# wgurecky/CORRLA_RS

Hardware: AMD Instinct MI355X
Metric: RSVD GFLOP/s on 16k x 16k f32 rank-128 (higher is better)
Workload: dtype f32

## Files before the change

corrla_rs_amd/csrc/driver.hpp:

```cpp
#pragma once
#include <cstdio>
#include <chrono>
#include <cmath>
#include <cstdint>
#include <cstring>
#include <limits>
#include <stdexcept>
#include <string>
#include <functional>
#include <vector>

#include "gemm_plan.hpp"
#include "small_linalg.hpp"

namespace corrla {

struct Error : std::runtime_error {
  int code;
  Error(int c, const std::string& m) : std::runtime_error(m), code(c) {}
};
enum { ST_OK = 0, ST_EINVAL = 1, ST_ENOMEM = 2, ST_EHIP = 3, ST_ECOMM = 4, ST_ENUMERIC = 5, ST_ENODEV = 6 };

inline int64_t round_up(int64_t x, int64_t a) { return (x + a - 1) / a * a; }

// ... 85 lines not shown
  bool qr_householder = false;
  static constexpr const T* kNone = nullptr;

  explicit RsvdDriver(Dev& d, bool profile = false) : dev(d), profile_phases(profile) {}

  int mixed_planes_ = 0;
  void a_times(const TallA<T>& a, const Skinny<T>& x, Skinny<T>& y, const T* scale_dev) {
    if (mixed_planes_ && dev.template mixed_fits<T>(!a.row_major, a.mem, x, y))
      dev.gemm_mixed(!a.row_major, a.mem, x, y, scale_dev, mixed_planes_), ++tm.n_mixed_products;
    else if (a.row_major)
      dev.gemm_nn(a.mem, x, y, scale_dev);
    else
      dev.gemm_tn(a.mem, x, y, scale_dev);
    if (a.mu_short || a.mu_tall) {
      T* v = dev.template alloc_scalar<T>((int)x.cols_alloc);
      dev.weighted_colsum(x, a.nt, a.mu_short, v);
      dev.rank1_sub(y, a.mt, a.mu_tall, v, scale_dev);
    }
  }
  void at_times(const TallA<T>& a, const Skinny<T>& y, Skinny<T>& z, const T* scale_dev, bool sharded) {
    if (mixed_planes_ && dev.template mixed_fits<T>(a.row_major, a.mem, y, z))
      dev.gemm_mixed(a.row_major, a.mem, y, z, scale_dev, mixed_planes_), ++tm.n_mixed_products;
    else if (a.row_major)
      dev.gemm_tn(a.mem, y, z, scale_dev);
    else
      dev.gemm_nn(a.mem, y, z, scale_dev);
    if (a.mu_short || a.mu_tall) {
      T* v = dev.template alloc_scalar<T>((int)y.cols_alloc);
      dev.weighted_colsum(y, a.mt, a.mu_tall, v);
      dev.rank1_sub(z, a.nt, a.mu_short, v, scale_dev);
    }
    if (sharded) dev.allreduce(z.p, (size_t)z.ld * (size_t)z.cols);
  }

  static constexpr size_t kStatusBytes = 32;
  int st_slots_ = 0;
  struct Pending {
    int slot, npass;
    bool rough;
    int per_pass;
    void* st = nullptr;
    int st_per_pass = 1;
    bool is_svd = false;
    int flag_slot = -1;
  };
  static constexpr int kRobustPasses = 8;
  bool robust_needs_more_ = false;
  bool svd_needs_more_ = false;
  bool svd_needs_v_ = false;
  bool null_cols_seen_ = false;
  int* flags_pool_ = nullptr;
  int flags_cap_ = 0, flags_used_ = 0;
  bool defer_status_ = false;
  bool optimistic_dirty_ = false;
  void* st_pool_ = nullptr;
  int st_used_ = 0;
  std::vector<Pending> pending_;
  int64_t m_local_ = 0, m_global_ = -1;
  int64_t m_local_override_ = -1;
  int64_t global_rows(bool sharded) {
    if (!sharded) return m_local_;
    if (m_global_ < 0) m_global_ = dev.allreduce_sum_host(m_local_);
    return m_global_;
  }

  int hh_short_shards_ = -1;
// ... 29 lines not shown
    if (const char* e = std::getenv("CORRLA_HH_BLOCK")) wmax = std::max<int64_t>(1, std::min<int64_t>(wmax, std::atoll(e)));
    if (l <= wmax) {
      householder_panel(y, tmp, sharded);
      return;
    }
    const int64_t nb = (l + wmax - 1) / wmax, w = (l + nb - 1) / nb;
    std::vector<double> th;
    for (int64_t c0 = 0; c0 < l; c0 += w) {
      const int64_t wb = std::min(w, l - c0);
      Skinny<T> yb = dev.template alloc_skinny<T>(m, wb), tb = dev.template alloc_skinny<T>(m, wb);
      Skinny<T> pb = dev.template alloc_skinny<T>(m, wb);
      dev.copy_block(y, 0, c0, m, wb, yb, 0, 0);
      for (int pass = 0; pass < 5; ++pass) {
        double overlap2 = 0.0;
        if (c0 > 0) {
          Skinny<T> t = dev.template alloc_skinny<T>(c0, wb);
          dev.gemm_nn(as_rowmajor_transposed(y, c0), yb, t, kNone);
          if (sharded) dev.allreduce(t.p, (size_t)t.ld * (size_t)t.cols_alloc);
          if (pass >= 1) {
            th.resize((size_t)(c0 * wb));
            dev.download_skinny(t, c0, wb, th.data());
            for (double v : th) overlap2 += v * v;
          }
          dev.gemm_tn(as_rowmajor_transposed(y, c0), t, pb, kNone);
          dev.sub_inplace(yb, pb);
        }
        householder_panel(yb, tb, sharded);
        if (c0 == 0 || (pass >= 1 && overlap2 <= 0.25)) break;
      }
      dev.copy_block(yb, 0, 0, m, wb, y, 0, c0);
    }
  }

  int64_t orthonormalize(Skinny<T>& y, Skinny<T>& tmp, bool sharded, bool rough = false) {
    const int64_t l = y.cols;
    if (householder_usable(y, sharded)) {
      PhaseTimer qt0;
      householder_thin_q_any_width(y, tmp, sharded);
      ++tm.qr_passes;
      subphase(tm.qr_gram_ms, qt0);
      return l;
    }
    int64_t r = orthonormalize_core(y, tmp, sharded, rough);
    if (r < l && !defer_status_ && (sharded ? global_rows(true) : y.rows) >= l) r = complete_basis(y, r, sharded);
    return r;
  }

  int64_t complete_basis(Skinny<T>& y, int64_t r, bool sharded) {
    const int64_t l = y.cols, c = l - r, m = y.rows;
    Skinny<T> yc = dev.template alloc_skinny<T>(m, c);
    Skinny<T> pc = dev.template alloc_skinny<T>(m, c);
    Skinny<T> tc = dev.template alloc_skinny<T>(m, c);
    dev.fill_normal(yc.p, m, c, (int64_t)1, yc.ld, (uint64_t)(0x9e3779b97f4a7c15ull ^ (uint64_t)(131 * r + l)), (int64_t)0, c);
    if (r > 0) {
      for (int pass = 0; pass < 2; ++pass) {
        Skinny<T> t = dev.template alloc_skinny<T>(r, c);
        dev.gemm_nn(as_rowmajor_transposed(y, r), yc, t, kNone);
        if (sharded) dev.allreduce(t.p, (size_t)t.ld * (size_t)t.cols_alloc);
        dev.gemm_tn(as_rowmajor_transposed(y, r), t, pc, kNone);
        dev.sub_inplace(yc, pc);
      }
    }
    const int64_t rc = orthonormalize_core(yc, tc, sharded, false);
    dev.copy_cols(yc, y, r, rc);
    return r + rc;
  }

  int64_t orthonormalize_device(Skinny<T>& y, Skinny<T>& tmp, bool sharded, bool rough, bool polish) {
    const int64_t l = y.cols;
    PhaseTimer qt0;
    const bool inplace = dev.qr_inplace_fits(l);
    const bool single = dev.template device_chol_fits<T>(l);
    const int level = std::max(2, std::min(dev.robust_passes(), kRobustPasses));
    const bool inloop = rough && !polish;
    const int npass_even = level;
    const int npass = inloop ? (level <= 2 ? 1 : npass_even - 1) : (polish ? (level <= 2 ? 1 : 3) : level);
    const int always = (polish || inloop) ? 1 : 2;
    int* need = flags_pool_ + flags_used_;
    int* null_mask = dev.alloc_flags((int)l);
    int* need_blk = dev.alloc_flags(2);
    void* st_scratch = dev.alloc_zeroed_bytes((size_t)2 * npass * kStatusBytes);
    void* insp = single ? nullptr : dev.template alloc_inspect<T>();
    Skinny<T> gd = dev.template alloc_skinny<T>(l, l);
    Skinny<T> md = dev.template alloc_skinny<T>(l, l);
    const double eps0 = (double)std::numeric_limits<T>::epsilon();
    double shift_rel = eps0 * std::max({16.0, 0.25 * std::sqrt((double)std::max<int64_t>(y.rows, 1)), single ? 0.0 : 2.0 * (double)l});
    if (const char* e = std::getenv("CORRLA_QR_SHIFT_SCALE")) shift_rel *= std::atof(e);
    float nullx = 1.f;
    if (const char* e = std::getenv("CORRLA_QR_NULL_EXCESS")) nullx = (float)std::atof(e);
    const int64_t n1 = single ? l : round_up((l + 1) / 2, (int64_t)4), n2 = l - n1;
    T* minus_one = nullptr;
    if (!single) {
      minus_one = dev.template alloc_scalar<T>(1);
      dev.fill_const(minus_one, (int64_t)1, (T)-1);
    }
    for (int pass = 0; pass < npass; ++pass) {
      const int gate = pass < always ? -1 : (inplace ? pass - 1 : always + ((pass - always) / 2) * 2 - 1);
      dev.set_run_if(gate < 0 ? nullptr : need + gate);
      Skinny<T> yv = y.view_cols(l);
      dev.gemm_nn(as_rowmajor_transposed(y, l), yv, gd, kNone);
      if (sharded) dev.allreduce(gd.p, (size_t)gd.ld * (size_t)gd.cols_alloc);
      const int shift_mode = polish ? 2 : (pass == 0 ? 1 : 0);
      const float nx = (!polish && pass >= 2) ? nullx : 0.f;
      const float need_ratio = (inloop && pass == 0) ? 1e-2f : 0.f;
      if (single) {
        dev.chol_inv_robust(gd, l, (T)(4.0 * eps0), (float)shift_rel, shift_mode, nx, md, st_scratch, pass, need + pass, null_mask,
                            nullptr, need_ratio);
      } else {
        dev.gram_inspect(gd, l, (float)shift_rel, shift_mode, insp);
        const void* shp = dev.template inspect_shift_ptr<T>(insp);
        Skinny<T> g11 = dev.template alloc_skinny<T>(n1, n1), g12 = dev.template alloc_skinny<T>(n1, n2);
        Skinny<T> g22 = dev.template alloc_skinny<T>(n2, n2), x11 = dev.template alloc_skinny<T>(n1, n1);
        Skinny<T> x22 = dev.template alloc_skinny<T>(n2, n2), r12 = dev.template alloc_skinny<T>(n1, n2);
        Skinny<T> t22 = dev.template alloc_skinny<T>(n2, n2), t12 = dev.template alloc_skinny<T>(n1, n2);
        Skinny<T> x12 = dev.template alloc_skinny<T>(n1, n2);
        dev.copy_block(gd, 0, 0, n1, n1, g11, 0, 0);
        dev.copy_block(gd, 0, n1, n1, n2, g12, 0, 0);
        dev.copy_block(gd, n1, n1, n2, n2, g22, 0, 0);
        dev.chol_inv_robust(g11, n1, (T)(4.0 * eps0), 0.f, 2, nx, x11, st_scratch, 2 * pass, need_blk, null_mask, shp, need_ratio);
        dev.gemm_nn(as_rowmajor_transposed(x11, n1), g12, r12, kNone);
        dev.gemm_nn(as_rowmajor_transposed(r12, n2), r12, t22, kNone);
        dev.sub_inplace(g22, t22);
        dev.chol_inv_robust(g22, n2, (T)(4.0 * eps0), 0.f, 2, nx, x22, st_scratch, 2 * pass + 1, need_blk + 1, null_mask + n1, shp,
                            need_ratio);
        dev.gemm_tn(as_rowmajor_transposed(r12, n2), x22, t12, kNone);
        dev.gemm_tn(as_rowmajor_transposed(x11, n1), t12, x12, minus_one);
        dev.copy_block(x11, 0, 0, n1, n1, md, 0, 0);
        dev.copy_block(x12, 0, 0, n1, n2, md, 0, n1);
        dev.copy_block(x22, 0, 0, n2, n2, md, n1, n1);
        dev.template combine_need<T>(need + pass, need_ratio > 0.f ? nullptr : insp, need_blk, need_blk + 1);
      }
      if (inplace) {
        dev.apply_inplace(y, l, md);
      } else {
        dev.gemm_tn(as_rowmajor_transposed(y, l), md, tmp, kNone);
        std::swap(y.p, tmp.p);
      }
      if (pass + 1 < npass || inloop) dev.refill_null(y, l, null_mask, (uint64_t)(0x9e3779b97f4a7c15ull ^ (uint64_t)(977 * (flags_used_ + pass) + l)));
      if (pass < always) ++tm.qr_passes;
    }
    dev.set_run_if(nullptr);
    Pending pd{always, npass, rough, 0};
    pd.st = st_scratch;
    pd.st_per_pass = single ? 1 : 2;
    pd.flag_slot = (inloop && npass > 1) ? -1 : flags_used_;
    pending_.push_back(pd);
    flags_used_ += npass;
    subphase(tm.qr_gram_ms, qt0);
    return l;
  }

  int64_t orthonormalize_core(Skinny<T>& y, Skinny<T>& tmp, bool sharded, bool rough, bool polish = false) {
    const int64_t l = y.cols;
    int64_t r = l;
    if (defer_status_ && (sharded || y.rows >= l) && flags_used_ + kRobustPasses <= flags_cap_ &&
        dev.template device_qr_robust_fits<T>(l))
      return orthonormalize_device(y, tmp, sharded, rough, polish);
    if (dev.template device_chol_fits<T>(l)) {
      PhaseTimer qt0;
      const int npass = rough ? 1 : 2;
      Skinny<T> gd0 = dev.template alloc_skinny<T>(l, l);
      Skinny<T> md0 = dev.template alloc_skinny<T>(l, l);
      const bool defer = defer_status_ && st_used_ + npass <= st_slots_;
      void* st_dev = defer ? (void*)((char*)st_pool_ + (size_t)st_used_ * kStatusBytes) : dev.alloc_bytes(2 * kStatusBytes);
      const double eps0 = (double)std::numeric_limits<T>::epsilon();
      for (int pass = 0; pass < npass; ++pass) {
        Skinny<T> yv = y.view_cols(l);
        dev.gemm_nn(as_rowmajor_transposed(y, l), yv, gd0, kNone);
        if (sharded) dev.allreduce(gd0.p, (size_t)gd0.ld * (size_t)gd0.cols_alloc);
        dev.chol_inv(gd0, l, (T)(4.0 * eps0), md0, st_dev, pass);
        dev.gemm_tn(as_rowmajor_transposed(y, l), md0, tmp, kNone);
        std::swap(y.p, tmp.p);
        ++tm.qr_passes;
      }
      if (defer) {
        pending_.push_back({st_used_, npass, rough, 1});
        st_used_ += npass;
        subphase(tm.qr_gram_ms, qt0);
        return l;
      }
      int fail[2] = {0, 0};
      float min_ratio[2], dev_i[2];
      dev.read_chol_status(st_dev, npass, fail, min_ratio, dev_i);
      subphase(tm.qr_gram_ms, qt0);
      for (int pass = 0; pass < npass; ++pass)
        if (fail[pass] == 3) throw Error(ST_ENUMERIC, "non-finite Gram matrix in orthonormalisation");
      if (fail[0] == 2) return 0;
      const bool ok = fail[0] == 0 && (rough || (fail[1] == 0 && dev_i[1] <= 0.25f));
      if (ok) return l;
    }
// ... 171 lines not shown
      dev.fill_normal(om.p, a.nt, l, 1, om.ld, o.seed, 0, l);
    }
    Skinny<T> z = dev.template alloc_skinny<T>(a.nt, l);
    double* ss_dev = dev.alloc_f64(1);
    T* inv_dev = dev.template alloc_scalar<T>(1);
    int64_t i0 = 0;
    const bool fused = o.power_fused && n_iter > 0 && a.row_major && !a.mu_short && !a.mu_tall &&
                       dev.template ata_fused_fits<T>(a.mem, l);
    if (fused) {
      const int64_t nf = std::min<int64_t>(n_iter, 3);
      for (int64_t i = 0; i < nf; ++i) {
        if (i == 0) dev.event_mark(0);
        dev.ata_fused(a.mem, i == 0 ? om : z, z);
        if (i == 0) dev.event_mark(1);
        if (o.sharded) dev.allreduce(z.p, (size_t)z.ld * (size_t)z.cols);
        dev.inv_norm(z, ss_dev, inv_dev);
        dev.scale_inplace(z, inv_dev);
        if (i == 0) phase(tm.sketch_ms, pt);
      }
      a_times(a, z, y, kNone);
      i0 = nf;
    } else {
      dev.event_mark(0);
      a_times(a, om, y, kNone);
      dev.event_mark(1);
      phase(tm.sketch_ms, pt);
    }
    for (int64_t i = i0; i < n_iter; ++i) {
      if (i > 2) {
        phase(tm.power_ms, pt);
        orthonormalize(y, y2, o.sharded, true);
        phase(tm.qr_ms, pt);
      }
      at_times(a, y, z, kNone, o.sharded);
      dev.inv_norm(z, ss_dev, inv_dev);
      dev.scale_inplace(z, inv_dev);
      a_times(a, z, y, kNone);
    }
    phase(tm.power_ms, pt);
    int64_t r = orthonormalize(y, y2, o.sharded);
    phase(tm.qr_ms, pt);
    return r;
  }

  void random_svd_tall(const TallA<T>& a, int64_t k, int64_t l, int64_t n_iter, const RunOpts& o, Skinny<T>& u_tall,
                       T* s_dev, Skinny<T>& v_tall, const std::function<void()>& emit = {}) {
    qr_householder = o.qr_householder;
    m_local_ = m_local_override_ >= 0 ? m_local_override_ : a.mt;
    m_global_ = -1;
    hh_short_shards_ = -1;
    const bool hh = qr_householder;
    if (!hh && (dev.template device_chol_fits<T>(l) || dev.template device_chol_blocked_fits<T>(l))) {
      const Timings saved = tm;
      const auto mark = dev.arena_mark();
      for (int attempt = 0; attempt < 5; ++attempt) {
        if (attempt > 0) dev.arena_rewind(mark);
        st_slots_ = (int)std::min<int64_t>(4 * (std::max<int64_t>(0, n_iter - 3) + 2) + 1, 4096);
        flags_cap_ = kRobustPasses * (int)std::min<int64_t>(std::max<int64_t>(0, n_iter - 3) + 4, 1024);
        st_pool_ = dev.alloc_zeroed_bytes((size_t)st_slots_ * kStatusBytes + (size_t)flags_cap_ * sizeof(int));
        st_used_ = 0;
        flags_pool_ = (int*)((char*)st_pool_ + (size_t)st_slots_ * kStatusBytes);
        flags_used_ = 0;
        pending_.clear();
        optimistic_dirty_ = false;
        robust_needs_more_ = false;
        svd_needs_more_ = false;
        svd_needs_v_ = false;
        null_cols_seen_ = false;
        defer_status_ = true;
        try {
// ... 86 lines not shown
        if (fail[(size_t)p.slot] == 1) {
          svd_needs_more_ = true;
          return false;
        }
        if (fail[(size_t)p.slot] == 4) {
          svd_needs_v_ = true;
          return false;
        }
      }
      for (int i = 0; i < p.npass * p.per_pass; ++i)
        if (fail[p.slot + i] != 0) return false;
      if (!p.rough)
        for (int i = 0; i < p.per_pass; ++i)
          if (!(dev_i[p.slot + (p.npass - 1) * p.per_pass + i] <= 0.25f)) return false;
    }
    return true;
  }

  void random_svd_tall_body(const TallA<T>& a, int64_t k, int64_t l, int64_t n_iter, const RunOpts& o, Skinny<T>& u_tall,
                            T* s_dev, Skinny<T>& v_tall) {
    PhaseTimer total;
    const bool hh_tmp = qr_householder;
    Skinny<T> q = dev.template alloc_skinny_out<T>(a.mt, l);
    Skinny<T> q2 = hh_tmp ? dev.template alloc_skinny<T>(a.mt, l) : dev.template alloc_skinny_out<T>(a.mt, l);
    power_iter(a, l, n_iter, o, q, q2);
    PhaseTimer pt;
    Skinny<T> bt = dev.template alloc_skinny<T>(a.nt, l);
    mixed_planes_ = o.mixed_project ? o.mixed_planes : 0;
    at_times(a, q, bt, kNone, o.sharded);
    mixed_planes_ = 0;
    phase(tm.project_ms, pt);
    Skinny<T> qb = dev.template alloc_skinny<T>(a.nt, l);
    Skinny<T> qb2 = dev.template alloc_skinny<T>(a.nt, l);
    dev.copy_skinny(bt, qb);
    orthonormalize(qb, qb2, false);
    phase(tm.qr_ms, pt);
    Skinny<T> ct = dev.template alloc_skinny<T>(l, l);
    dev.gemm_nn(as_rowmajor_transposed(bt, l), qb, ct, kNone);
    if (o.poison_core) dev.poison_entry(ct, l / 2, l / 3, o.poison_core);
    Skinny<T> m1 = dev.template alloc_skinny<T>(l, k);
    Skinny<T> m2 = dev.template alloc_skinny<T>(l, k);
    void* svd_st = nullptr;
    if (defer_status_ && st_used_ + 1 <= st_slots_) {
      svd_st = (void*)((char*)st_pool_ + (size_t)st_used_ * kStatusBytes);
      pending_.push_back({st_used_, 1, true, 1});
      pending_.back().is_svd = true;
      st_used_ += 1;
    }
    dev.small_svd(ct, l, k, m2, m1, s_dev, svd_st);
    int64_t nz_known = k;
    if (defer_status_) {
      Skinny<T> m1b = dev.template alloc_skinny<T>(l, k);
      orthonormalize_core(m1, m1b, false, true, true);
    }
    if (!defer_status_) {
      std::vector<T> sh((size_t)k);
      dev.copy_values_out(s_dev, k, sh.data(), true);
      const T null_tol = (T)(1e-3 * (double)std::numeric_limits<T>::epsilon()) * sh[0];
      int64_t nz = 0;
      while (nz < k && sh[(size_t)nz] > null_tol) ++nz;
      if (nz < k) complete_basis(m1, nz, false);
      nz_known = nz;
      if (nz == k) {
        Skinny<T> m1b = dev.template alloc_skinny<T>(l, k);
        orthonormalize_core(m1, m1b, false, true);
      }
    }
    (void)nz_known;
// ... 79 lines not shown
```

corrla_rs_amd/csrc/hip_backend.hpp:

```cpp
#pragma once
#include <hip/hip_runtime.h>
#include <rccl/rccl.h>

#include <cmath>
#include <cstdio>
#include <cstdlib>
#include <cstring>
#include <limits>
#include <random>
#include <string>
#include <type_traits>
#include <vector>

#include "core_svd_plan.hpp"
#include "driver.hpp"
#include "hip_kernels.hpp"
#include "tsqr_kernels.hpp"
#include "jacobi_mc_kernels.hpp"
#include "ata_kernels.hpp"
#include "tall_kernels.hpp"
#include "mixed_kernels.hpp"
#include "grad_kernels.hpp"
#include "knn2_kernels.hpp"
#include "grad_wide_kernels.hpp"
// ... 105 lines not shown
    return z ? z : 0x5eedull;
  }

  void comm_init(const void* id128, int rank, int nranks_) {
    CORRLA_HIP(hipSetDevice(device));
    ncclUniqueId id;
    static_assert(sizeof(ncclUniqueId) <= CORRLA_UNIQUE_ID_BYTES, "unique id size");
    std::memcpy(&id, id128, sizeof(id));
    if (comm) {
      (void)ncclCommDestroy(comm);
      comm = nullptr;
    }
    CORRLA_NCCL(ncclCommInitRank(&comm, nranks_, id, rank));
    comm_rank = rank;
    comm_size = nranks_;
  }
  void comm_info(int* rank_out, int* nranks_out) {
    if (!comm) {
      *rank_out = 0;
      *nranks_out = 0;
      return;
    }
    CORRLA_NCCL(ncclCommUserRank(comm, rank_out));
    CORRLA_NCCL(ncclCommCount(comm, nranks_out));
  }

  void begin_call() {
    CORRLA_HIP(hipSetDevice(device));
    events_set_[0] = events_set_[1] = events_set_[2] = false;
    n_collectives = 0;
    collective_bytes = 0;
    marks_.clear();
    ev_used_ = 0;
    phase_mark(nullptr);
    for (auto& c : chunks_) c.used = 0;
    for (auto& c : zchunks_) {
      c.zeroed = std::min<size_t>(c.used, (size_t)256 << 20);
      c.used = 0;
      if (c.zeroed) CORRLA_HIP(hipMemsetAsync(c.p, 0, c.zeroed, stream));
    }
  }
  void end_call() { sync(); }
  void sync() { CORRLA_HIP(hipStreamSynchronize(stream)); }

  void* alloc_bytes(size_t bytes) {
    bytes = (bytes + 255) / 256 * 256;
    if (bytes == 0) bytes = 256;
    for (auto& c : chunks_)
      if (c.size - c.used >= bytes) {
        void* p = (char*)c.p + c.used;
        c.used += bytes;
        return p;
      }
    Chunk c;
    c.size = std::max<size_t>(bytes, (size_t)64 << 20);
    if (hipMalloc(&c.p, c.size) != hipSuccess) {
      (void)hipGetLastError();
      throw Error(ST_ENOMEM, "device allocation of " + std::to_string(c.size) + " bytes failed");
    }
    c.used = bytes;
    chunks_.push_back(c);
    return c.p;
  }
  void memset_zero(void* p, size_t bytes) { CORRLA_HIP(hipMemsetAsync(p, 0, bytes, stream)); }
  void* alloc_zeroed(size_t bytes) {
    bytes = (bytes + 255) / 256 * 256;
// ... 556 lines not shown
    jmc_local_ = env_int("CORRLA_JMC_LOCAL", 1);
    const int lanes = jmc_lanes<T>(l);
    const int rp = k::jmc_pitch(nc, (int)sizeof(T), lanes), nblocks = 2 * np, ncols_pad = nblocks * b;
    T* wj = (T*)alloc_bytes((size_t)rp * ncols_pad * sizeof(T));
    T* vj = (T*)alloc_bytes((size_t)rp * ncols_pad * sizeof(T));
    k::JmcCtl* ctl = (k::JmcCtl*)alloc_bytes(sizeof(k::JmcCtl));
    k::CholStatus* st = conv_status ? (k::CholStatus*)conv_status : (k::CholStatus*)alloc_bytes(sizeof(k::CholStatus));
    const int force_v = (conv_status == nullptr || jmc_force_v_ || env_int("CORRLA_JMC_FORCE_V", 0)) ? 1 : 0;
    hipLaunchKernelGGL((k::jmc_init_kernel<T>), dim3(1), dim3(1024), 0, stream, (const T*)c.p, c.ld, (int)l, wj, vj, rp,
                       ncols_pad, force_v, ctl);
    const double eps = (double)std::numeric_limits<T>::epsilon();
    const T tol = (T)(std::sqrt((double)l) * eps);
    const T tol_early = env_int("CORRLA_JACOBI_STRICT", 0) ? tol : (T)std::sqrt(eps);
    const T floor2 = (T)((double)l * eps * eps);
    auto enqueue_sweeps = [&](int s0, int s1) {
      for (int sw = s0; sw < s1; ++sw)
        for (int step = 0; step < nblocks - 1; ++step) switch (nc) {
            case 1: jmc_launch_step<T, 1>(lanes, np, b, wj, vj, nblocks, step, sw, tol, tol_early, floor2, ctl); break;
            case 2: jmc_launch_step<T, 2>(lanes, np, b, wj, vj, nblocks, step, sw, tol, tol_early, floor2, ctl); break;
            case 3: jmc_launch_step<T, 3>(lanes, np, b, wj, vj, nblocks, step, sw, tol, tol_early, floor2, ctl); break;
            case 4: jmc_launch_step<T, 4>(lanes, np, b, wj, vj, nblocks, step, sw, tol, tol_early, floor2, ctl); break;
            case 5: jmc_launch_step<T, 5>(lanes, np, b, wj, vj, nblocks, step, sw, tol, tol_early, floor2, ctl); break;
            case 6: jmc_launch_step<T, 6>(lanes, np, b, wj, vj, nblocks, step, sw, tol, tol_early, floor2, ctl); break;
            case 7: jmc_launch_step<T, 7>(lanes, np, b, wj, vj, nblocks, step, sw, tol, tol_early, floor2, ctl); break;
            case 8: jmc_launch_step<T, 8>(lanes, np, b, wj, vj, nblocks, step, sw, tol, tol_early, floor2, ctl); break;
            default: jmc_launch_step<T, 9>(lanes, np, b, wj, vj, nblocks, step, sw, tol, tol_early, floor2, ctl); break;
          }
      CORRLA_HIP(hipGetLastError());
    };
    const size_t lds_fin = (size_t)(l + 2) * sizeof(T) + (size_t)(l + 2) * sizeof(int) + 64;
    auto finish = [&](int nsw) {
      hipLaunchKernelGGL((k::jmc_finish_kernel<T>), dim3(1), dim3(1024), lds_fin, stream, (const T*)wj, (const T*)vj, rp, (int)l,
                         nsw, (const k::JmcCtl*)ctl, m1.p, m1.ld, m2.p, m2.ld, s_dev, (int)k, st);
      const unsigned groups = (unsigned)(l * k);
      hipLaunchKernelGGL((k::jmc_other_factor_kernel<T>), dim3((groups * 16 + 255) / 256), dim3(256), 0, stream, (const T*)c.p,
                         c.ld, (int)l, (int)k, (const T*)m2.p, m2.ld, (const T*)s_dev, (const k::JmcCtl*)ctl, m1.p, m1.ld);
      CORRLA_HIP(hipGetLastError());
    };
    if (conv_status) {
      const int nsw_default = std::max(1, env_int("CORRLA_JMC_SWEEPS", sizeof(T) == 4 ? 10 : 13));
      const int nsw = std::min(k::kJmcMaxSweeps, (jmc_sweeps_hint_ > 0 ? std::min(nsw_default, jmc_sweeps_hint_ + 2) : nsw_default) + jmc_extra_sweeps_);
      enqueue_sweeps(0, nsw);
      finish(nsw);
      if (env_int("CORRLA_DEBUG", 0)) {
        k::JmcCtl hd;
        CORRLA_HIP(hipMemcpyAsync(&hd, ctl, sizeof(hd), hipMemcpyDeviceToHost, stream));
        sync();
        int used = 0;
        while (used < nsw && hd.rot[used] && hd.big[used]) ++used;
        std::fprintf(stderr, "[corrla] jacobi_svd (multi-workgroup, %d sweeps enqueued, %s) l=%d np=%d b=%d nc=%d sweeps run=%d rounds(wg0)=%llu "
                             "cycles/round=%.0f ns/round=%.0f (%.0f MHz)\n", nsw, hd.with_v ? "V accumulated" : "W only", (int)l, np, b, nc, std::min(used + 1, nsw),
                     hd.rounds, hd.rounds ? (double)hd.clk / hd.rounds : 0.0, hd.rounds ? 10.0 * hd.wall / hd.rounds : 0.0,
                     hd.wall ? 100.0 * hd.clk / hd.wall : 0.0);
        if (hd.steps)
          std::fprintf(stderr, "[corrla]   per step (wg0, us): load %.2f norms %.2f rounds %.2f store %.2f total %.2f over %llu steps\n",
                       0.01 * hd.t_load / hd.steps, 0.01 * hd.t_norm / hd.steps, 0.01 * hd.wall / hd.steps,
                       0.01 * hd.t_store / hd.steps, 0.01 * hd.t_total / hd.steps, hd.steps);
        if (hd.steps > 1)
          std::fprintf(stderr, "[corrla]   span first-start..last-end over all workgroups: %.2f us per step\n",
                       0.01 * hd.t_span / (hd.steps - 1));
      }
      return;
    }
    int done = 0;
    k::JmcCtl h;
    while (done < k::kJmcMaxSweeps) {
      const int s1 = std::min(k::kJmcMaxSweeps, done + 8);
      enqueue_sweeps(done, s1);
      CORRLA_HIP(hipMemcpyAsync(&h, ctl, sizeof(h), hipMemcpyDeviceToHost, stream));
      sync();
      bool conv = false;
      for (int s_ = 0; s_ < s1; ++s_) conv = conv || !(h.rot[s_] && h.big[s_]);
      done = s1;
      if (conv || h.bad) break;
    }
    if (h.bad) throw Error(ST_ENUMERIC, "non-finite core matrix in small SVD");
    finish(done);
    if (env_int("CORRLA_DEBUG", 0)) {
      int used = 0;
      while (used < done && h.rot[used] && h.big[used]) ++used;
      std::fprintf(stderr, "[corrla] jacobi_svd (multi-workgroup) l=%d np=%d b=%d sweeps=%d\n", (int)l, np, b, used + 1);
    }
  }

  template <class T>
  void small_svd(const Skinny<T>& c, int64_t l, int64_t k, Skinny<T>& m1, Skinny<T>& m2, T* s_dev, void* conv_status) {
    if (conv_status) memset_zero(conv_status, sizeof(k::CholStatus));
    CoreSvdKnobs kn;
    kn.mode = std::getenv("CORRLA_SVD");
    kn.host_svd = env_int("CORRLA_HOST_SVD", 0) != 0;
    kn.jmc_min_l = jmc_min_l_;
    kn.jmc_max_b = jmc_max_b_;
    kn.jmc_local = env_int("CORRLA_JMC_LOCAL", 1);
    kn.jmc_np = env_int("CORRLA_JMC_NP", 0);
    const CoreSvdPlan plan = core_svd_plan((int)sizeof(T), l, kn);
    switch (plan.family) {
      case CoreSvd::kMultiWg:
        small_svd_mc(c, l, k, m1, m2, s_dev, conv_status);
        return;
      case CoreSvd::kHost:
        small_svd_host(*this, c, l, k, m1, m2, s_dev);
        return;
      case CoreSvd::kBlock:
        core_finite_check<T>(c, l, conv_status);
        small_svd_block(c, l, k, m1, m2, s_dev);
        return;
      case CoreSvd::kRing:
        core_finite_check<T>(c, l, conv_status);
        small_svd_ring(c, l, k, m1, m2, s_dev, plan.ring_e);
        return;
    }
  }
  template <class T>
  void core_finite_check(const Skinny<T>& c, int64_t l, void* conv_status) {
    int* bad = conv_status ? nullptr : alloc_flags(1);
    hipLaunchKernelGGL((k::core_finite_check_kernel<T>), dim3(1), dim3(1024), 0, stream, (const T*)c.p, c.ld, (int)l,
                       (k::CholStatus*)conv_status, bad);
    CORRLA_HIP(hipGetLastError());
    if (bad) {
      int h = 0;
      read_flags(bad, 1, &h);
      if (h) throw Error(ST_ENUMERIC, "non-finite core matrix in small SVD");
    }
  }

  template <class T>
  void small_svd_block(const Skinny<T>& c, int64_t l, int64_t k, Skinny<T>& m1, Skinny<T>& m2, T* s_dev) {
    const int nb = (int)(2 * ((l + 15) / 16));
// ... 109 lines not shown
    CORRLA_HIP(hipGetLastError());
  }

  template <class T>
  void fix_signs(Skinny<T>& v_ref, Skinny<T>& other, int64_t k) {
    hipLaunchKernelGGL((k::column_sign_apply_kernel<T>), dim3((unsigned)k), dim3(256), 0, stream, v_ref.p, v_ref.ld, v_ref.rows,
                       other.p, other.ld, other.rows);
    CORRLA_HIP(hipGetLastError());
  }
  template <class T>
  void fill_const(T* p, int64_t n, T v) {
    const int blocks = (int)std::min<int64_t>(2048, std::max<int64_t>(1, (n + 255) / 256));
    hipLaunchKernelGGL((k::fill_const_kernel<T>), dim3(blocks), dim3(256), 0, stream, p, n, v);
    CORRLA_HIP(hipGetLastError());
  }
  template <class T>
  void center_rows_cols(const T* in, int64_t rows, int64_t cols, int64_t ldi, const T* mu, bool along_cols, T* out,
                        int64_t ldo) {
    dim3 grid((unsigned)((cols + 255) / 256), (unsigned)std::min<int64_t>(rows, 4096));
    hipLaunchKernelGGL((k::center_kernel<T>), grid, dim3(256), 0, stream, in, rows, cols, ldi, mu, along_cols ? 1 : 0, out,
                       ldo);
    CORRLA_HIP(hipGetLastError());
  }

  template <class T>
  void sumsq(const Skinny<T>& y, double* out_dev) {
    const int64_t n = y.ld * y.cols_alloc;
    const int blocks = (int)std::min<int64_t>(1024, std::max<int64_t>(1, (n + 255) / 256));
    double* partial = (double*)alloc_bytes(sizeof(double) * blocks);
    hipLaunchKernelGGL((k::sumsq_partial_kernel<T>), dim3(blocks), dim3(256), 0, stream, y.p, n, partial);
    hipLaunchKernelGGL(k::sum_partials_kernel, dim3(1), dim3(64), 0, stream, partial, blocks, out_dev);
    CORRLA_HIP(hipGetLastError());
  }
  template <class T>
  void inv_norm(const Skinny<T>& y, double* ss_dev, T* inv_dev) {
    const int64_t n = y.ld * y.cols_alloc;
    const int blocks = (int)std::min<int64_t>(1024, std::max<int64_t>(1, (n + 255) / 256));
    double* partial = (double*)alloc_bytes(sizeof(double) * blocks);
    hipLaunchKernelGGL((k::sumsq_partial_kernel<T>), dim3(blocks), dim3(256), 0, stream, y.p, n, partial);
    hipLaunchKernelGGL((k::sum_partials_rsqrt_kernel<T>), dim3(1), dim3(64), 0, stream, (const double*)partial, blocks, ss_dev, inv_dev);
    CORRLA_HIP(hipGetLastError());
  }
  template <class T>
  void rsqrt_scalar(const double* ss_dev, T* out_dev) {
    hipLaunchKernelGGL((k::rsqrt_scalar_kernel<T>), dim3(1), dim3(1), 0, stream, ss_dev, out_dev);
    CORRLA_HIP(hipGetLastError());
  }
  template <class T>
  void scale_inplace(Skinny<T>& y, const T* scale_dev) {
    const int64_t n = y.ld * y.cols_alloc;
    const int blocks = (int)std::min<int64_t>(2048, std::max<int64_t>(1, (n + 255) / 256));
    hipLaunchKernelGGL((k::scale_kernel<T>), dim3(blocks), dim3(256), 0, stream, y.p, n, scale_dev);
    CORRLA_HIP(hipGetLastError());
  }
  template <class T>
  void fill_normal(T* p, int64_t rows, int64_t cols, int64_t rs, int64_t cs, uint64_t seed, int64_t row0,
                   int64_t global_cols) {
    const int64_t n = rows * cols;
    if (n <= 0) return;
    const int blocks = (int)std::min<int64_t>(8192, (n + 255) / 256);
    hipLaunchKernelGGL((k::fill_normal_kernel<T>), dim3(blocks), dim3(256), 0, stream, p, rows, cols, rs, cs, seed, row0,
                       global_cols, cs <= rs ? 1 : 0);
    CORRLA_HIP(hipGetLastError());
  }

  void set_phase_events(bool on) { phase_events_ = on; }
  void phase_end() {
    if (!phase_events_) phase_mark_impl(nullptr);
// ... 66 lines not shown
  }

 private:
  struct Chunk {
    void* p = nullptr;
    size_t size = 0, used = 0;
    size_t zeroed = 0;
  };
  std::vector<Chunk> chunks_;
  std::vector<Chunk> zchunks_;
  void* zero_page_ = nullptr;
  void* pinned_ = nullptr;
  hipEvent_t events_[3] = {nullptr, nullptr, nullptr};
  bool events_set_[3] = {false, false, false};
  struct PhaseMark {
    hipEvent_t ev;
    double* slot;
  };
  std::vector<hipEvent_t> ev_pool_;
  size_t ev_used_ = 0;
  std::vector<PhaseMark> marks_;
  static constexpr size_t kPinnedBytes = (size_t)8 << 20;
  int gemm_debug_flags_ = 0;
  GemmKnobs gemm_knobs_;
  uint64_t entropy_ = 0, calls_ = 0, calls_sharded_ = 0;
  bool no_device_chol_ = false;
  int jmc_min_l_ = 96, jmc_max_b_ = 24, jmc_local_ = 1;
  const int* run_if_ = nullptr;
  bool phase_events_ = true;
  bool robust_qr_ = true;
  int robust_passes_ = 2;
  int jmc_extra_sweeps_ = 0, jmc_sweeps_hint_ = 0;
  bool jmc_force_v_ = false;

  static void check_grid(const dim3& g) {
    if (g.y > 65535u || g.z > 65535u) throw Error(ST_EINVAL, "problem too large for the launch grid");
  }

  static void lds_limit(const void* fn, size_t bytes) {
    CORRLA_HIP(hipFuncSetAttribute(fn, hipFuncAttributeMaxDynamicSharedMemorySize, (int)bytes));
  }
  static void set_lds_limits() {
    constexpr size_t kMax = k::kLdsMaxBytes;
    set_lds_limits_typed<float>();
    set_lds_limits_typed<double>();
    set_ata_limits<2>();
    set_ata_limits<4>();
    set_ata_limits<8>();
    set_mixed_limits<2, false>();
    set_mixed_limits<2, true>();
    set_mixed_limits<3, false>();
    set_mixed_limits<3, true>();
    lds_limit((const void*)k::knn_kernel, kMax);
    lds_limit((const void*)k::knn_mfma_kernel<4, 4>, kMax);
    lds_limit((const void*)k::knn_mfma_kernel<4, 8>, kMax);
    lds_limit((const void*)k::knn_mfma_kernel<4, 16>, kMax);
    lds_limit((const void*)k::knn_mfma_kernel<2, 4>, kMax);
    lds_limit((const void*)k::knn_mfma_kernel<2, 8>, kMax);
    lds_limit((const void*)k::knn_mfma_kernel<2, 16>, kMax);
    lds_limit((const void*)k::knn2_kernel<1>, k::k2_lds_bytes(1));
    lds_limit((const void*)k::knn2_kernel<2>, k::k2_lds_bytes(2));
    lds_limit((const void*)k::grad_fit_kernel, kMax);
    lds_limit((const void*)k::grad_fit_lin_kernel<1>, kMax);
    lds_limit((const void*)k::grad_fit_lin_kernel<2>, kMax);
    lds_limit((const void*)k::grad_fit_lin_kernel<3>, kMax);
    lds_limit((const void*)k::grad_fit_lin_kernel<4>, kMax);
// ... 51 lines not shown
    auto aligned = [](const void* p) { return (uintptr_t)p % 16 == 0; };
    GemmShape s;
    s.tn = tn;
    s.esz = (int)sizeof(T);
    s.r = {r.rows, r.cols, r.ld, r.cols_readable, 0, false, aligned(r.p)};
    s.x = {x.rows, x.cols, x.ld, 0, x.cols_alloc, x.external, aligned(x.p)};
    s.out = {out.rows, out.cols, out.ld, 0, out.cols_alloc, out.external, aligned(out.p)};
    s.same = (const void*)r.p == (const void*)x.p;
    s.np = np;
    s.num_cus = num_cus;
    return s;
  }
  template <class T>
  GemmPlan plan_gemm(bool tn, const Big<T>& r, const Skinny<T>& x, const Skinny<T>& out, int np) const {
    const GemmPlan p = gemm_plan(gemm_shape(tn, r, x, out, np), gemm_knobs_);
    if (p.error) throw Error(ST_EINVAL, p.error);
    return p;
  }
  template <int MAX, int N = 1, class F>
  static void with_nt(int n, const F& f) {
    if constexpr (N < MAX) {
      if (n > N) return with_nt<MAX, N + 1>(n, f);
    }
    if (n != N) throw Error(ST_EINVAL, "internal: no kernel instantiation for " + std::to_string(n));
    f(std::integral_constant<int, N>{});
  }
  template <int MAX, int N = 1, class F>
  static void for_each_nt(const F& f) {
    f(std::integral_constant<int, N>{});
    if constexpr (N < MAX) for_each_nt<MAX, N + 1>(f);
  }
  template <class T>
  void slab_reduce(const SlabReducePlan& rp, const T* slab, int64_t stride, T* out, int64_t ld, const T* scale, const int* run_if) {
    if (rp.kind == SlabReduce::none) return;
    const dim3 grid(rp.grid[0], rp.grid[1]);
    if (rp.kind == SlabReduce::deep)
      hipLaunchKernelGGL((k::slab_reduce_deep_kernel<T>), grid, dim3(256), 0, stream, slab, stride, rp.slabs, out, ld, rp.rows,
                         rp.cols, scale, run_if);
    else
      hipLaunchKernelGGL((k::slab_reduce_kernel<T>), grid, dim3(256), 0, stream, slab, stride, rp.slabs, out, ld, rp.rows, rp.cols,
                         scale, run_if);
    CORRLA_HIP(hipGetLastError());
  }

  template <class T, int NT>
  void launch_general(bool tn, const GemmPlan& p, dim3 grid, dim3 block, int lds, const k::GemmArgs<T>& a) {
    with_nt<2>(p.mw, [&](auto mw) {
      with_nt<8, 4>(p.nw, [&](auto nw) {
        constexpr int MW = decltype(mw)::value, NW = decltype(nw)::value;
        if constexpr (NW == 4 || (NW == 8 && MW == 1 && std::is_same<T, double>::value)) {
          if (tn)
            hipLaunchKernelGGL((k::gemm_tn_kernel<T, MW, NT, NW>), grid, block, lds, stream, a);
          else
            hipLaunchKernelGGL((k::gemm_nn_kernel<T, MW, NT, false, NW>), grid, block, lds, stream, a);
        }
      });
    });
  }

  template <class T>
  void launch_gemm(bool tn, const Big<T>& r, const Skinny<T>& x, Skinny<T>& out, const T* scale_dev) {
    const GemmPlan p = plan_gemm(tn, r, x, out, 0);
    const GemmLaunch& L0 = p.launch[0];
    T* slab = p.reduce.kind != SlabReduce::none ? (T*)alloc_bytes(p.slab_bytes) : nullptr;
    if (p.family == GemmFamily::tall_apply) {
      const k::TallApplyArgs<T> g{r.p, r.cols, r.ld, (int)r.rows, x.p, x.ld, (int)x.cols, out.p, out.ld, (int)p.out_cols,
                                  scale_dev, p.vec_store, run_if_};
      with_nt<sizeof(T) == 4 ? 6 : 4>(L0.nt, [&](auto kt) {
        constexpr int K = decltype(kt)::value;
// ... 45 lines not shown
```

corrla_rs_amd/csrc/hip_kernels.hpp:

```cpp
#pragma once
#include <hip/hip_runtime.h>

#include <limits>
#include <stdint.h>

#include <type_traits>

#include "gemm_plan.hpp"

namespace corrla {
namespace k {

typedef float f32x4 __attribute__((ext_vector_type(4)));
typedef double f64x4 __attribute__((ext_vector_type(4)));
typedef double f64x2 __attribute__((ext_vector_type(2)));

#ifndef CORRLA_F32_BIG_IS_A
#define CORRLA_F32_BIG_IS_A true
#endif
template <class T>
struct MT;
template <>
struct MT<float> {
  typedef f32x4 acc_t;
// ... 604 lines not shown
  for (int ob = 0; ob < nob; ++ob, n0 += ob_cols) {
#pragma unroll
    for (int mw = 0; mw < MW; ++mw)
#pragma unroll
      for (int t = 0; t < NT; ++t) acc[mw][t] = (acc_t){0, 0, 0, 0};
    for (int i = 0; i < nk; ++i) {
      wg_barrier();
      compute(buf, i > 0);
      buf = buf + 1 == gemm_stages(GW, NT) ? 0 : buf + 1;
    }
    if constexpr (kDefer > 0) {
      if (nk > 0) static_for<NS - kDefer, NS>(mfma_step);
    }
#pragma unroll
    for (int mw = 0; mw < MW; ++mw)
      store_tile<T, NT>(g, acc[mw], n0 + 16 * MW * wave + 16 * mw, g.r_cols, col0, lane, bz);
  }
}

template <class T>
__global__ void slab_reduce_kernel(const T* slab, int64_t slab_stride, int nsplit, T* out, int64_t ld, int64_t limit,
                                   int64_t ncols, const T* scale, const int* run_if = nullptr) {
  if (run_if && *run_if == 0) return;
  const int64_t i = (int64_t)blockIdx.x * blockDim.x + threadIdx.x;
  const int64_t col = blockIdx.y;
  if (i >= limit || col >= ncols) return;
  const int64_t off = col * ld + i;
  T s = 0;
  for (int z = 0; z < nsplit; ++z) s += slab[(int64_t)z * slab_stride + off];
  if (scale) s *= *scale;
  out[off] = s;
}
template <class T>
__global__ __launch_bounds__(256) void slab_reduce_deep_kernel(const T* slab, int64_t slab_stride, int nsplit, T* out,
                                                               int64_t ld, int64_t limit, int64_t ncols, const T* scale,
                                                               const int* run_if = nullptr) {
  if (run_if && *run_if == 0) return;
  __shared__ T part[4][64];
  const int li = threadIdx.x & 63, zg = threadIdx.x >> 6;
  const int64_t i = (int64_t)blockIdx.x * 64 + li;
  const int64_t col = blockIdx.y;
  const int per = (nsplit + 3) / 4;
  const int z0 = zg * per, z1 = min(nsplit, z0 + per);
  T s0 = 0, s1 = 0, s2 = 0, s3 = 0;
  if (i < limit && col < ncols) {
    const T* src = slab + col * ld + i;
    int z = z0;
    for (; z + 3 < z1; z += 4) {
      s0 += src[(int64_t)z * slab_stride];
      s1 += src[(int64_t)(z + 1) * slab_stride];
      s2 += src[(int64_t)(z + 2) * slab_stride];
      s3 += src[(int64_t)(z + 3) * slab_stride];
    }
    for (; z < z1; ++z) s0 += src[(int64_t)z * slab_stride];
  }
  part[zg][li] = (s0 + s1) + (s2 + s3);
  __syncthreads();
  if (zg == 0 && i < limit && col < ncols) {
    T s = (part[0][li] + part[1][li]) + (part[2][li] + part[3][li]);
    if (scale) s *= *scale;
    out[col * ld + i] = s;
  }
}

template <class T>
__global__ void sumsq_partial_kernel(const T* y, int64_t n, double* partial) {
  double s = 0.0;
  for (int64_t i = (int64_t)blockIdx.x * blockDim.x + threadIdx.x; i < n; i += (int64_t)gridDim.x * blockDim.x) {
    const double v = (double)y[i];
    s += v * v;
  }
  for (int off = 32; off > 0; off >>= 1) s += __shfl_down(s, off, 64);
  __shared__ double ws[4];
  if ((threadIdx.x & 63) == 0) ws[threadIdx.x >> 6] = s;
  __syncthreads();
  if (threadIdx.x == 0) partial[blockIdx.x] = ws[0] + ws[1] + ws[2] + ws[3];
}
__global__ void sum_partials_kernel(const double* partial, int n, double* out) {
  double s = 0.0;
  for (int i = threadIdx.x; i < n; i += 64) s += partial[i];
  for (int off = 32; off > 0; off >>= 1) s += __shfl_down(s, off, 64);
  if (threadIdx.x == 0) *out = s;
}
template <class T>
__global__ void sum_partials_rsqrt_kernel(const double* partial, int n, double* ss_out, T* inv_out) {
  double s = 0.0;
  for (int i = threadIdx.x; i < n; i += 64) s += partial[i];
  for (int off = 32; off > 0; off >>= 1) s += __shfl_down(s, off, 64);
  if (threadIdx.x == 0) {
    *ss_out = s;
    *inv_out = (T)(s > 0.0 ? 1.0 / sqrt(s) : 0.0);
  }
}
template <class T>
__global__ void rsqrt_scalar_kernel(const double* ss, T* out) {
  const double v = *ss;
  *out = (T)(v > 0.0 ? 1.0 / sqrt(v) : 0.0);
}
template <class T>
__global__ void sub_kernel(T* y, const T* __restrict__ p, int64_t n) {
  for (int64_t i = (int64_t)blockIdx.x * blockDim.x + threadIdx.x; i < n; i += (int64_t)gridDim.x * blockDim.x) y[i] -= p[i];
}
template <class T>
__global__ void scale_kernel(T* y, int64_t n, const T* scale) {
  const T sc = *scale;
  for (int64_t i = (int64_t)blockIdx.x * blockDim.x + threadIdx.x; i < n; i += (int64_t)gridDim.x * blockDim.x)
    y[i] *= sc;
}

__device__ __forceinline__ void philox4x32_10(uint32_t (&c)[4], uint32_t k0, uint32_t k1) {
#pragma unroll
  for (int r = 0; r < 10; ++r) {
    const uint64_t p0 = (uint64_t)0xD2511F53u * c[0];
    const uint64_t p1 = (uint64_t)0xCD9E8D57u * c[2];
    const uint32_t n0 = (uint32_t)(p1 >> 32) ^ c[1] ^ k0;
    const uint32_t n1 = (uint32_t)p1;
    const uint32_t n2 = (uint32_t)(p0 >> 32) ^ c[3] ^ k1;
    const uint32_t n3 = (uint32_t)p0;
    c[0] = n0;
    c[1] = n1;
// ... 1210 lines not shown
```

Baseline: 94200.

## Fuse norm into slab reduce, fold scaling into GEMM, skip copies in QR

In the power iteration, the split-K slab reduction after A^T*Y can now accumulate sum-of-squares partials, so inv_norm only runs a tiny final reduction instead of rereading Z. The explicit scale_inplace is replaced by passing the inverse norm as the GEMM scale in the non-sharded path. Orthonormalization accepts a source matrix, so the first Gram pass and the first apply read directly from bt and the copy into qb is dropped. The multi-WG SVD path also skips a redundant status memset and one factor kernel when V is forced. Together these remove extra memory passes and kernel launches, at the cost of more code paths and a stateful arm/consume norm protocol.

```diff
diff --git a/corrla_rs_amd/csrc/driver.hpp b/corrla_rs_amd/csrc/driver.hpp
--- a/corrla_rs_amd/csrc/driver.hpp
+++ b/corrla_rs_amd/csrc/driver.hpp
@@ -141,6 +141,13 @@
     }
     if (sharded) dev.allreduce(z.p, (size_t)z.ld * (size_t)z.cols);
   }
+
+  template <class D>
+  static auto arm_product_norm(D& d, int) -> decltype(d.arm_product_norm(), void()) {
+    d.arm_product_norm();
+  }
+  template <class D>
+  static void arm_product_norm(D&, long) {}
 
   static constexpr size_t kStatusBytes = 32;
   int st_slots_ = 0;
@@ -236,16 +243,17 @@
     }
   }
 
-  int64_t orthonormalize(Skinny<T>& y, Skinny<T>& tmp, bool sharded, bool rough = false) {
+  int64_t orthonormalize(Skinny<T>& y, Skinny<T>& tmp, bool sharded, bool rough = false, const Skinny<T>* src = nullptr) {
     const int64_t l = y.cols;
     if (householder_usable(y, sharded)) {
+      if (src) dev.copy_skinny(*src, y);
       PhaseTimer qt0;
       householder_thin_q_any_width(y, tmp, sharded);
       ++tm.qr_passes;
       subphase(tm.qr_gram_ms, qt0);
       return l;
     }
-    int64_t r = orthonormalize_core(y, tmp, sharded, rough);
+    int64_t r = orthonormalize_core(y, tmp, sharded, rough, false, src);
     if (r < l && !defer_status_ && (sharded ? global_rows(true) : y.rows) >= l) r = complete_basis(y, r, sharded);
     return r;
   }
@@ -270,7 +278,8 @@
     return r + rc;
   }
 
-  int64_t orthonormalize_device(Skinny<T>& y, Skinny<T>& tmp, bool sharded, bool rough, bool polish) {
+  int64_t orthonormalize_device(Skinny<T>& y, Skinny<T>& tmp, bool sharded, bool rough, bool polish,
+                                const Skinny<T>* src = nullptr) {
     const int64_t l = y.cols;
     PhaseTimer qt0;
     const bool inplace = dev.qr_inplace_fits(l);
@@ -301,8 +310,10 @@
     for (int pass = 0; pass < npass; ++pass) {
       const int gate = pass < always ? -1 : (inplace ? pass - 1 : always + ((pass - always) / 2) * 2 - 1);
       dev.set_run_if(gate < 0 ? nullptr : need + gate);
-      Skinny<T> yv = y.view_cols(l);
-      dev.gemm_nn(as_rowmajor_transposed(y, l), yv, gd, kNone);
+      const bool from_src = pass == 0 && src != nullptr;
+      const Skinny<T>& in = from_src ? *src : y;
+      Skinny<T> yv = in.view_cols(l);
+      dev.gemm_nn(as_rowmajor_transposed(in, l), yv, gd, kNone);
       if (sharded) dev.allreduce(gd.p, (size_t)gd.ld * (size_t)gd.cols_alloc);
       const int shift_mode = polish ? 2 : (pass == 0 ? 1 : 0);
       const float nx = (!polish && pass >= 2) ? nullx : 0.f;
@@ -334,10 +345,12 @@
         dev.copy_block(x22, 0, 0, n2, n2, md, n1, n1);
         dev.template combine_need<T>(need + pass, need_ratio > 0.f ? nullptr : insp, need_blk, need_blk + 1);
       }
-      if (inplace) {
+      if (from_src && inplace) {
+        dev.gemm_tn(as_rowmajor_transposed(in, l), md, y, kNone);
+      } else if (inplace) {
         dev.apply_inplace(y, l, md);
       } else {
-        dev.gemm_tn(as_rowmajor_transposed(y, l), md, tmp, kNone);
+        dev.gemm_tn(as_rowmajor_transposed(in, l), md, tmp, kNone);
         std::swap(y.p, tmp.p);
       }
       if (pass + 1 < npass || inloop) dev.refill_null(y, l, null_mask, (uint64_t)(0x9e3779b97f4a7c15ull ^ (uint64_t)(977 * (flags_used_ + pass) + l)));
@@ -354,12 +367,14 @@
     return l;
   }
 
-  int64_t orthonormalize_core(Skinny<T>& y, Skinny<T>& tmp, bool sharded, bool rough, bool polish = false) {
+  int64_t orthonormalize_core(Skinny<T>& y, Skinny<T>& tmp, bool sharded, bool rough, bool polish = false,
+                              const Skinny<T>* src = nullptr) {
     const int64_t l = y.cols;
     int64_t r = l;
     if (defer_status_ && (sharded || y.rows >= l) && flags_used_ + kRobustPasses <= flags_cap_ &&
         dev.template device_qr_robust_fits<T>(l))
-      return orthonormalize_device(y, tmp, sharded, rough, polish);
+      return orthonormalize_device(y, tmp, sharded, rough, polish, src);
+    if (src) dev.copy_skinny(*src, y);
     if (dev.template device_chol_fits<T>(l)) {
       PhaseTimer qt0;
       const int npass = rough ? 1 : 2;
@@ -597,10 +612,15 @@
         orthonormalize(y, y2, o.sharded, true);
         phase(tm.qr_ms, pt);
       }
+      if (!o.sharded && !a.mu_short && !a.mu_tall) arm_product_norm(dev, 0);
       at_times(a, y, z, kNone, o.sharded);
       dev.inv_norm(z, ss_dev, inv_dev);
-      dev.scale_inplace(z, inv_dev);
-      a_times(a, z, y, kNone);
+      if (o.sharded) {
+        dev.scale_inplace(z, inv_dev);
+        a_times(a, z, y, kNone);
+      } else {
+        a_times(a, z, y, inv_dev);
+      }
     }
     phase(tm.power_ms, pt);
     int64_t r = orthonormalize(y, y2, o.sharded);
@@ -753,8 +773,7 @@
     phase(tm.project_ms, pt);
     Skinny<T> qb = dev.template alloc_skinny<T>(a.nt, l);
     Skinny<T> qb2 = dev.template alloc_skinny<T>(a.nt, l);
-    dev.copy_skinny(bt, qb);
-    orthonormalize(qb, qb2, false);
+    orthonormalize(qb, qb2, false, false, &bt);
     phase(tm.qr_ms, pt);
     Skinny<T> ct = dev.template alloc_skinny<T>(l, l);
     dev.gemm_nn(as_rowmajor_transposed(bt, l), qb, ct, kNone);
diff --git a/corrla_rs_amd/csrc/hip_backend.hpp b/corrla_rs_amd/csrc/hip_backend.hpp
--- a/corrla_rs_amd/csrc/hip_backend.hpp
+++ b/corrla_rs_amd/csrc/hip_backend.hpp
@@ -161,6 +161,8 @@
     collective_bytes = 0;
     marks_.clear();
     ev_used_ = 0;
+    norm_armed_ = false;
+    norm_out_ = nullptr;
     phase_mark(nullptr);
     for (auto& c : chunks_) c.used = 0;
     for (auto& c : zchunks_) {
@@ -783,6 +785,10 @@
     auto finish = [&](int nsw) {
       hipLaunchKernelGGL((k::jmc_finish_kernel<T>), dim3(1), dim3(1024), lds_fin, stream, (const T*)wj, (const T*)vj, rp, (int)l,
                          nsw, (const k::JmcCtl*)ctl, m1.p, m1.ld, m2.p, m2.ld, s_dev, (int)k, st);
+      if (force_v) {
+        CORRLA_HIP(hipGetLastError());
+        return;
+      }
       const unsigned groups = (unsigned)(l * k);
       hipLaunchKernelGGL((k::jmc_other_factor_kernel<T>), dim3((groups * 16 + 255) / 256), dim3(256), 0, stream, (const T*)c.p,
                          c.ld, (int)l, (int)k, (const T*)m2.p, m2.ld, (const T*)s_dev, (const k::JmcCtl*)ctl, m1.p, m1.ld);
@@ -836,7 +842,6 @@
 
   template <class T>
   void small_svd(const Skinny<T>& c, int64_t l, int64_t k, Skinny<T>& m1, Skinny<T>& m2, T* s_dev, void* conv_status) {
-    if (conv_status) memset_zero(conv_status, sizeof(k::CholStatus));
     CoreSvdKnobs kn;
     kn.mode = std::getenv("CORRLA_SVD");
     kn.host_svd = env_int("CORRLA_HOST_SVD", 0) != 0;
@@ -845,6 +850,7 @@
     kn.jmc_local = env_int("CORRLA_JMC_LOCAL", 1);
     kn.jmc_np = env_int("CORRLA_JMC_NP", 0);
     const CoreSvdPlan plan = core_svd_plan((int)sizeof(T), l, kn);
+    if (conv_status && plan.family != CoreSvd::kMultiWg) memset_zero(conv_status, sizeof(k::CholStatus));
     switch (plan.family) {
       case CoreSvd::kMultiWg:
         small_svd_mc(c, l, k, m1, m2, s_dev, conv_status);
@@ -1020,8 +1026,16 @@
     hipLaunchKernelGGL(k::sum_partials_kernel, dim3(1), dim3(64), 0, stream, partial, blocks, out_dev);
     CORRLA_HIP(hipGetLastError());
   }
+  void arm_product_norm() { norm_armed_ = true; }
   template <class T>
   void inv_norm(const Skinny<T>& y, double* ss_dev, T* inv_dev) {
+    if (norm_out_ == (const void*)y.p) {
+      norm_out_ = nullptr;
+      hipLaunchKernelGGL((k::sum_partials_rsqrt_kernel<T>), dim3(1), dim3(64), 0, stream, (const double*)norm_partial_, norm_n_, ss_dev,
+                         inv_dev);
+      CORRLA_HIP(hipGetLastError());
+      return;
+    }
     const int64_t n = y.ld * y.cols_alloc;
     const int blocks = (int)std::min<int64_t>(1024, std::max<int64_t>(1, (n + 255) / 256));
     double* partial = (double*)alloc_bytes(sizeof(double) * blocks);
@@ -1154,6 +1168,10 @@
   int robust_passes_ = 2;
   int jmc_extra_sweeps_ = 0, jmc_sweeps_hint_ = 0;
   bool jmc_force_v_ = false;
+  bool norm_armed_ = false;
+  const void* norm_out_ = nullptr;
+  double* norm_partial_ = nullptr;
+  int norm_n_ = 0;
 
   static void check_grid(const dim3& g) {
     if (g.y > 65535u || g.z > 65535u) throw Error(ST_EINVAL, "problem too large for the launch grid");
@@ -1271,9 +1289,19 @@
   }
   template <class T>
   void slab_reduce(const SlabReducePlan& rp, const T* slab, int64_t stride, T* out, int64_t ld, const T* scale, const int* run_if) {
+    const bool want_norm = norm_armed_;
+    norm_armed_ = false;
+    norm_out_ = nullptr;
     if (rp.kind == SlabReduce::none) return;
     const dim3 grid(rp.grid[0], rp.grid[1]);
-    if (rp.kind == SlabReduce::deep)
+    if (want_norm && rp.kind == SlabReduce::plain && !run_if) {
+      const unsigned gy = std::max(1u, std::min(rp.grid[1], 2048u / std::max(1u, rp.grid[0])));
+      norm_n_ = (int)(rp.grid[0] * gy);
+      norm_partial_ = (double*)alloc_bytes(sizeof(double) * (size_t)norm_n_);
+      hipLaunchKernelGGL((k::slab_reduce_sumsq_kernel<T>), dim3(rp.grid[0], gy), dim3(256), 0, stream, slab, stride, rp.slabs, out, ld,
+                         rp.rows, rp.cols, scale, norm_partial_);
+      norm_out_ = out;
+    } else if (rp.kind == SlabReduce::deep)
       hipLaunchKernelGGL((k::slab_reduce_deep_kernel<T>), grid, dim3(256), 0, stream, slab, stride, rp.slabs, out, ld, rp.rows,
                          rp.cols, scale, run_if);
     else
diff --git a/corrla_rs_amd/csrc/hip_kernels.hpp b/corrla_rs_amd/csrc/hip_kernels.hpp
--- a/corrla_rs_amd/csrc/hip_kernels.hpp
+++ b/corrla_rs_amd/csrc/hip_kernels.hpp
@@ -660,6 +660,28 @@
   out[off] = s;
 }
 template <class T>
+__global__ __launch_bounds__(256) void slab_reduce_sumsq_kernel(const T* slab, int64_t slab_stride, int nsplit, T* out, int64_t ld,
+                                                                int64_t limit, int64_t ncols, const T* scale, double* partial) {
+  const int64_t i = (int64_t)blockIdx.x * blockDim.x + threadIdx.x;
+  double ss = 0.0;
+  if (i < limit) {
+    for (int64_t col = blockIdx.y; col < ncols; col += gridDim.y) {
+      const int64_t off = col * ld + i;
+      T s = 0;
+      for (int z = 0; z < nsplit; ++z) s += slab[(int64_t)z * slab_stride + off];
+      if (scale) s *= *scale;
+      out[off] = s;
+      const double v = (double)s;
+      ss += v * v;
+    }
+  }
+  for (int off = 32; off > 0; off >>= 1) ss += __shfl_down(ss, off, 64);
+  __shared__ double ws[4];
+  if ((threadIdx.x & 63) == 0) ws[threadIdx.x >> 6] = ss;
+  __syncthreads();
+  if (threadIdx.x == 0) partial[(int64_t)blockIdx.y * gridDim.x + blockIdx.x] = ws[0] + ws[1] + ws[2] + ws[3];
+}
+template <class T>
 __global__ __launch_bounds__(256) void slab_reduce_deep_kernel(const T* slab, int64_t slab_stride, int nsplit, T* out,
                                                                int64_t ld, int64_t limit, int64_t ncols, const T* scale,
                                                                const int* run_if = nullptr) {
@@ -713,7 +735,14 @@
 template <class T>
 __global__ void sum_partials_rsqrt_kernel(const double* partial, int n, double* ss_out, T* inv_out) {
   double s = 0.0;
-  for (int i = threadIdx.x; i < n; i += 64) s += partial[i];
+  for (int i0 = threadIdx.x; i0 < n; i0 += 8 * 64) {
+    double xb[8];
+#pragma unroll
+    for (int u = 0; u < 8; ++u) xb[u] = partial[min(i0 + 64 * u, n - 1)];
+#pragma unroll
+    for (int u = 0; u < 8; ++u)
+      if (i0 + 64 * u < n) s += xb[u];
+  }
   for (int off = 32; off > 0; off >>= 1) s += __shfl_down(s, off, 64);
   if (threadIdx.x == 0) {
     *ss_out = s;
```

Measured after the change: 93700. Within noise of the previous version (-0.5%).
